# Avirup221/Multimodal-Hierarchical-CNN-for-Sun-Salutation-Pose-Classification

Hardware: AMD Instinct MI355X
Metric: images/sec fwd+bwd QuadtreeCNN 224x224 bs256 (higher is better)
Workload: dtype bf16; 1 GPU; QuadtreeCNN (ResNet-18 layer3, 2x2 split, 47-feat fusion) train step fwd+bwd+Adam, all parameters trainable; Adam(lr 1e-4, wd 1e-4) by the package's FusedAdam (csrc/pack.hip); global_batch=256, per_gpu_batch=256, image=3x224x224, num_classes=12, parallelism=dp1

## Files before the change

include/qtcnn.h:

```cpp
#ifndef QTCNN_H_
#define QTCNN_H_

#include <stddef.h>
#include <stdint.h>

#ifdef __cplusplus
extern "C" {
#endif

typedef enum qt_status {
  QT_OK = 0,
  QT_ERR_INVALID_ARG = -1,
  QT_ERR_LAUNCH = -2,
  QT_ERR_UNSUPPORTED = -3
} qt_status;

typedef enum qt_dtype { QT_F32 = 0, QT_BF16 = 1 } qt_dtype;

int qt_version(void);
const char* qt_last_error(void);

enum { QT_CONV_FWD = 0, QT_CONV_DGRAD = 1 };

typedef struct qt_conv_desc {
// ... 398 lines not shown
int qt_pack_dgrad_s2_merged(int dtype, const float* w_oihw, void* dst, int O, int I, void* stream);
int qt_pack_stem_weight(int dtype, const float* w_oihw, void* dst, int taps, void* stream);
int qt_unpack_conv_wgrad(const float* dw, float* grad_oihw, int O, int I, int kh, int kw, int accumulate, void* stream);
int qt_unpack_stem_wgrad(const float* dw, float* grad_oihw, int accumulate, void* stream);

int qt_stats_capacity_rows(int rows);
int qt_bn_finalize(float* partial, int rows, int C, long long count, const float* gamma, const float* beta,
                   float* running_mean, float* running_var, long long* num_batches_tracked, float momentum, float eps,
                   float* mean, float* invstd, float* scale, float* shift, void* stream);
int qt_bn_eval_affine(const float* gamma, const float* beta, const float* running_mean, const float* running_var,
                      float eps, int C, float* scale, float* shift, void* stream);
typedef struct qt_bn_eval_item {
  const float *gamma, *beta, *running_mean, *running_var;
  float *scale, *shift;
  int C;
  float *mean, *invstd;
} qt_bn_eval_item;
int qt_bn_eval_affine_batched(const qt_bn_eval_item* items, int n, float eps, void* stream);
int qt_bn_act(int dtype, const void* y, const float* scale, const float* shift, const void* residual,
              const float* res_scale, const float* res_shift, int relu, void* out, long long M, int C, void* stream);
int qt_bn_act_mask(int dtype, const void* y, const float* scale, const float* shift, const void* residual,
                   const float* res_scale, const float* res_shift, int relu, void* out, unsigned char* mask_bits,
                   long long M, int C, void* stream);
int qt_bn_bwd_partial_rows(long long M, int C);
int qt_bn_bwd_reduce(int dtype, const void* g, const void* mask, const void* y, const float* mean, const float* invstd,
                     float* partial, long long M, int C, void* stream);
int qt_bn_bwd_finalize(float* partial, int rows, int C, long long count, const float* gamma, const float* invstd,
                       float* dgamma, float* dbeta, int accumulate, float* coef , void* stream);
int qt_bn_bwd_apply(int dtype, const void* g, const void* mask, const void* y, const float* mean, const float* invstd,
                    const float* coef, void* dy, void* g_out, long long M, int C, void* stream);

int qt_stem_pool(int dtype, const void* y, const float* scale, const float* shift, void* pooled,
                 unsigned char* argmax, void* y_at_max, int batch, void* stream);
int qt_stem_conv_pool(int dtype, const void* xpad, const void* weight, int taps, const float* scale, const float* shift,
                      void* pooled, int batch, void* stream);
int qt_stem_conv_pool_nchw(int dtype, const float* image_nchw, const void* weight, int taps, const float* scale,
                           const float* shift, void* pooled, int batch, void* stream);
int qt_stem_pool_bwd(int dtype, const void* dpooled, const unsigned char* argmax, const void* y, const float* scale,
                     const float* shift, void* g, int batch, void* stream);
int qt_stem_bn_bwd_rows(int batch);
int qt_stem_bn_bwd_reduce(int dtype, const void* dpooled, const unsigned char* argmax, const void* y,
                          const float* scale, const float* shift, const float* mean, const float* invstd,
                          float* partial, int batch, void* stream);
int qt_stem_bn_bwd_sums_rows(int batch);
int qt_stem_bn_bwd_sums(int dtype, const void* dpooled, const void* y_at_max, const float* scale, const float* shift,
                        const float* mean, const float* invstd, float* partial, int batch, void* stream);
int qt_stem_bn_bwd_apply(int dtype, const void* dpooled, const unsigned char* argmax, const void* y, const float* scale,
                         const float* shift, const float* mean, const float* invstd, const float* coef, void* dy,
                         int batch, void* stream);
size_t qt_stem_bn_bwd_wgrad_workspace_bytes(int batch);
int qt_stem_bn_bwd_wgrad_ws(int dtype, const void* dpooled, const unsigned char* argmax, const void* y, const float* scale,
                            const float* shift, const float* mean, const float* invstd, const float* coef, const void* xpad,
                            float* dw, void* workspace, size_t workspace_bytes, int batch, void* stream);
int qt_stem_dgrad(int dtype, const void* dy, const float* w_oihw, float* dx, int batch, void* stream);
int qt_avgpool(int dtype, const void* x, void* dst, int batch, int hw, int C, int ld, int col0, void* stream);
int qt_avgpool_bwd(int dtype, const void* d, const void* x, void* g, int batch, int hw, int C, int ld, int col0,
                   void* stream);
int qt_quad_pool(int dtype, const void* q, void* dst, int batch, int ld, int col0, void* stream);
int qt_quad_pool_bwd(int dtype, const void* d, const void* q, void* dq, int batch, int ld, int col0, void* stream);
int qt_region_avgpool(int dtype, const void* x, void* dst, int dst_dtype, int batch, int split, int hw, int C, int ld,
                      int col0, void* stream);
int qt_region_avgpool_bwd(int dtype, const void* d, int d_dtype, const void* x, void* g, int batch, int split, int hw,
                          int C, int ld, int col0, void* stream);
int qt_attention_gate(int dtype, const float* v, const float* w1, const float* b1, const float* w2, const float* b2,
                      float* act, float* alpha, void* out, int batch, int ld, int col0, void* stream);
int qt_attention_gate_bwd(int dtype, const void* d, const float* v, const float* act, const float* alpha, const float* w1,
                          const float* w2, float* ds, float* dpre, float* dv, int batch, int ld, int col0, void* stream);
int qt_relu_mask_cols(int dtype, const void* d, const void* act, float* out, long long rows, int cols, int ld, int col0,
                      float mul, void* stream);
int qt_lstm_forward(const float* xproj, const float* whh_t, const float* bhh, float* gates, float* cell, float* hprev,
// ... 139 lines not shown
```

multimodal-hierarchical-cnn-for-sun-salutation-pose-classification_amd/csrc/conv_stem.hip:

```cpp
#include <stdlib.h>

#include "qt_internal.h"

namespace {

struct StemArgs {
  const bf16_t* x;
  const bf16_t* w;
  bf16_t* y;
  const float* scale;
  const float* shift;
  float* stats;
  int relu, taps, ntiles;
};

constexpr int ST_TH = 4;
constexpr int ST_ROWB = QT_STEM_PAD_W * 4 * 2;
constexpr int ST_IN_ROWS = 2 * ST_TH + 5;
constexpr int ST_BUF = 24 * 1024;
static_assert(ST_IN_ROWS * ST_ROWB <= ST_BUF, "a tile's input rows fit one buffer");
constexpr int ST_STG_ROW = 144;
constexpr int ST_STG = 16 * ST_STG_ROW;
constexpr int ST_LDS = 2 * ST_BUF + 4 * ST_STG;

template <bool AFF, bool STATS>
__global__ __launch_bounds__(256) void conv_stem_kernel(StemArgs p) {
  extern __shared__ __attribute__((aligned(16))) unsigned char smem[];
  const int tid = threadIdx.x, lane = tid & 63;
  const int wave = __builtin_amdgcn_readfirstlane(tid >> 6);
  const int li = lane & 15, lg = lane >> 4;
  const unsigned smem_base = lds_addr_of(smem);

  const int t_beg = (int)((long long)blockIdx.x * p.ntiles / gridDim.x);
  const int t_end = (int)((long long)(blockIdx.x + 1) * p.ntiles / gridDim.x);

  uint4 wf[7][4];
#pragma unroll
  for (int kh = 0; kh < 7; ++kh)
#pragma unroll
    for (int cb = 0; cb < 4; ++cb)
      wf[kh][cb] = *reinterpret_cast<const uint4*>(p.w + ((size_t)(cb * 16 + li) * p.taps + kh) * 32 + lg * 8);

  float sc[4][4], sh[4][4];
#pragma unroll
  for (int cb = 0; cb < 4; ++cb)
#pragma unroll
    for (int r = 0; r < 4; ++r) {
      const int ch = cb * 16 + lg * 4 + r;
      sc[cb][r] = p.scale ? p.scale[ch] : 1.f;
      sh[cb][r] = p.scale ? p.shift[ch] : 0.f;
    }
  float s1[4][4], s2[4][4];
#pragma unroll
  for (int cb = 0; cb < 4; ++cb)
#pragma unroll
    for (int r = 0; r < 4; ++r) s1[cb][r] = s2[cb][r] = 0.f;

  auto dma_tile = [&](int tile, int buf) {
    const int img = tile / 28, rg = tile - img * 28;
    const unsigned char* src = reinterpret_cast<const unsigned char*>(p.x) +
                               ((size_t)img * QT_STEM_PAD_H + (size_t)rg * 2 * ST_TH) * ST_ROWB;
#pragma unroll
    for (int i = 0; i < 6; ++i) {
      const int blk = wave * 6 + i;
      glds16(src + blk * 1024 + lane * 16, smem_base + buf * ST_BUF + blk * 1024);
    }
  };

  unsigned char* stg = smem + 2 * ST_BUF + wave * ST_STG;
  const unsigned keep8 = lg == 3 ? 0u : 0xffffffffu;
  if (t_beg < t_end) dma_tile(t_beg, 0);
  for (int t = t_beg; t < t_end; ++t) {
    const int buf = (t - t_beg) & 1;
    asm volatile("s_waitcnt vmcnt(0)\n\ts_barrier" ::: "memory");
    if (t + 1 < t_end) dma_tile(t + 1, buf ^ 1);
    const unsigned char* in = smem + buf * ST_BUF;
    const int img = t / 28, rg = t - img * 28;
#pragma unroll 1
    for (int j = 0; j < 7; ++j) {
      const int rb = wave + 4 * j;
      const int orow = rb / 7, ob = rb - orow * 7;
      const unsigned char* a0 = in + (2 * orow) * ST_ROWB + 16 * (ob * 16 + li + lg);
      uint4 xf[7];
#pragma unroll
      for (int kh = 0; kh < 7; ++kh) {
        xf[kh] = *reinterpret_cast<const uint4*>(a0 + kh * ST_ROWB);
        xf[kh].z &= keep8;
        xf[kh].w &= keep8;
      }
      f32x4 acc[4];
#pragma unroll
      for (int cb = 0; cb < 4; ++cb) acc[cb] = (f32x4){0.f, 0.f, 0.f, 0.f};
      __builtin_amdgcn_s_setprio(1);
#pragma unroll
      for (int kh = 0; kh < 7; ++kh)
#pragma unroll
        for (int cb = 0; cb < 4; ++cb)
          acc[cb] = __builtin_amdgcn_mfma_f32_16x16x32_bf16(__builtin_bit_cast(bf16x8, wf[kh][cb]),
                                                            __builtin_bit_cast(bf16x8, xf[kh]), acc[cb], 0, 0, 0);
      __builtin_amdgcn_s_setprio(0);
#pragma unroll
      for (int cb = 0; cb < 4; ++cb) {
        float v[4];
#pragma unroll
        for (int r = 0; r < 4; ++r) {
          const float a = acc[cb][r];
          if (STATS) {
            s1[cb][r] += a;
// ... 215 lines not shown
      auto max4 = [&](const uint4& a, const uint4& b) -> uint4 {
        return make_uint4(pkmax(a.x, b.x), pkmax(a.y, b.y), pkmax(a.z, b.z), pkmax(a.w, b.w));
      };
      const uint4 zero = make_uint4(0u, 0u, 0u, 0u);
      uint4 raw[5][3];
#pragma unroll
      for (int tr = 0; tr < 5; ++tr)
#pragma unroll
        for (int dc = 0; dc < 3; ++dc) {
          const int col = 2 * pw - 1 + dc;
          raw[tr][dc] = zero;
          if (!(k == 0 && tr == 0) && (unsigned)col < 112u)
            raw[tr][dc] = *reinterpret_cast<const uint4*>(ctile + (tr * 112 + col) * SP_PXB + cg * 16);
        }
      uint4 rowmax[5];
#pragma unroll
      for (int tr = 0; tr < 5; ++tr) rowmax[tr] = max4(max4(raw[tr][0], raw[tr][1]), raw[tr][2]);
#pragma unroll
      for (int pi = 0; pi < 2; ++pi) {
        const uint4 best = max4(max4(rowmax[2 * pi], rowmax[2 * pi + 1]), rowmax[2 * pi + 2]);
        *reinterpret_cast<uint4*>(p.pooled + (((size_t)img * 56 + 2 * k + pi) * 56 + pw) * 64 + cg * 8) = best;
      }
    }
  }
  asm volatile("s_waitcnt vmcnt(0)" ::: "memory");
}

int g_stem_enabled = -1;
bool stem_enabled() {
  if (g_stem_enabled < 0) g_stem_enabled = qt_env_int("QTCNN_STEM_CONV", 1);
  return g_stem_enabled != 0;
}

int stem_grid(int batch) {
  const int ntiles = batch * (112 / ST_TH);
  return ntiles < 512 ? ntiles : 512;
}

}

extern "C" void qt_set_stem_conv(int mode) { g_stem_enabled = mode < 0 ? 1 : (mode != 0); }

bool qt_stem_eligible(const qt_conv_desc* d, const qt_conv_io* io) {
  if (!stem_enabled() || d->dtype != QT_BF16 || d->mode != QT_CONV_FWD) return false;
  if (d->k_per_tap != 32 || d->kw != 1 || (d->kh != 7 && d->kh != 8) || d->stride != 2 || d->pad != 0) return false;
  if (d->n_out != 64 || d->out_h != 112 || d->out_w != 112 || d->in_h != QT_STEM_PAD_H || d->in_w != QT_STEM_PAD_W)
    return false;
  if (d->src_pix_stride != 4 || d->src_row_stride != QT_STEM_PAD_W * 4 ||
      d->src_img_stride != (long long)QT_STEM_PAD_H * QT_STEM_PAD_W * 4)
    return false;
  if (d->quad || d->dst_sub) return false;
  if (io && (io->residual || io->relu_mask || io->relu_mask_bits || io->bwd_bn[0].y || io->bwd_bn[1].y)) return false;
  return true;
}

int qt_stem_stats_rows(const qt_conv_desc* d) { return stem_grid(d->batch); }

int qt_stem_launch(const qt_conv_desc* d, const qt_conv_io* io, void* stream) {
  QT_CHECK_ARG((io->scale == nullptr) == (io->shift == nullptr), "qt_conv2d_igemm: scale and shift come together");
  StemArgs a;
  a.x = static_cast<const bf16_t*>(io->src);
  a.w = static_cast<const bf16_t*>(io->weight);
  a.y = static_cast<bf16_t*>(io->dst);
  a.scale = io->scale; a.shift = io->shift; a.stats = io->stats_partial;
  a.relu = d->relu; a.taps = d->kh; a.ntiles = d->batch * (112 / ST_TH);
  const bool aff = a.scale != nullptr || a.relu, stats = a.stats != nullptr;
  void (*kern)(StemArgs) = aff ? (stats ? conv_stem_kernel<true, true> : conv_stem_kernel<true, false>)
                               : (stats ? conv_stem_kernel<false, true> : conv_stem_kernel<false, false>);
  static std::atomic<unsigned long long> lds_limit_set[4];
  const int ki = (aff ? 2 : 0) + (stats ? 1 : 0);
  if (int rc = qt_raise_lds_limit(reinterpret_cast<const void*>(kern), ST_LDS, lds_limit_set[ki])) return rc;
  hipLaunchKernelGGL(kern, dim3(stem_grid(d->batch)), dim3(256), ST_LDS, static_cast<hipStream_t>(stream), a);
  QT_CHECK_LAUNCH();
  return QT_OK;
}

extern "C" int qt_stem_conv_pool(int dtype, const void* xpad, const void* weight, int taps, const float* scale,
                                 const float* shift, void* pooled, int batch, void* stream) {
  QT_CHECK_ARG(xpad && weight && scale && shift && pooled && batch > 0 && (taps == 7 || taps == 8),
               "qt_stem_conv_pool: bad argument");
  if (dtype != QT_BF16 || !stem_enabled()) {
    qt_set_error("qt_stem_conv_pool: bf16 only (use qt_conv2d_igemm + qt_stem_pool)");
    return QT_ERR_UNSUPPORTED;
  }
  StemPoolArgs a;
  a.x = static_cast<const bf16_t*>(xpad); a.w = static_cast<const bf16_t*>(weight); a.img = nullptr;
  a.pooled = static_cast<bf16_t*>(pooled); a.scale = scale; a.shift = shift; a.taps = taps; a.ntiles = batch * 28;
  static std::atomic<unsigned long long> lds_limit_set{0};
  if (int rc = qt_raise_lds_limit(reinterpret_cast<const void*>(conv_stem_pool_kernel<false>), SP_LDS, lds_limit_set)) return rc;
  const int grid = a.ntiles < 256 ? a.ntiles : 256;
  hipLaunchKernelGGL(conv_stem_pool_kernel<false>, dim3(grid), dim3(512), SP_LDS, static_cast<hipStream_t>(stream), a);
  QT_CHECK_LAUNCH();
  return QT_OK;
}

extern "C" int qt_stem_conv_pool_nchw(int dtype, const float* image_nchw, const void* weight, int taps, const float* scale,
                                      const float* shift, void* pooled, int batch, void* stream) {
  QT_CHECK_ARG(image_nchw && weight && scale && shift && pooled && batch > 0 && (taps == 7 || taps == 8),
               "qt_stem_conv_pool_nchw: bad argument");
  static const int raw_on = qt_env_int("QTCNN_STEM_NCHW", 1);
  if (dtype != QT_BF16 || !stem_enabled() || !raw_on || ((uintptr_t)image_nchw % 16) != 0) {
    qt_set_error("qt_stem_conv_pool_nchw: bf16 and a 16-byte aligned image only (use qt_pack_stem_input + qt_stem_conv_pool)");
    return QT_ERR_UNSUPPORTED;
  }
  StemPoolArgs a;
  a.x = nullptr; a.img = image_nchw; a.w = static_cast<const bf16_t*>(weight);
  a.pooled = static_cast<bf16_t*>(pooled); a.scale = scale; a.shift = shift; a.taps = taps; a.ntiles = batch * 28;
  static std::atomic<unsigned long long> lds_limit_set{0};
  if (int rc = qt_raise_lds_limit(reinterpret_cast<const void*>(conv_stem_pool_kernel<true>), SP_LDS_RAW, lds_limit_set)) return rc;
// ... 6 lines not shown
```

multimodal-hierarchical-cnn-for-sun-salutation-pose-classification_amd/csrc/elementwise.hip:

```cpp
#include "qt_common.h"

namespace {

__device__ __forceinline__ void load8f(const float* p, float (&v)[8]) { QtVec8<float>::load(p, v); }

constexpr int kFinC = 16;

__device__ __forceinline__ void sum_partial_rows(const float* __restrict__ partial, int rows, int C, int c, int rl,
                                                 double& s1, double& s2) {
  int r = rl;
  for (; r + 16 * 7 < rows; r += 16 * 8) {
    float a[8], b[8];
#pragma unroll
    for (int k = 0; k < 8; ++k) {
      a[k] = partial[((long long)(r + 16 * k) * 2 + 0) * C + c];
      b[k] = partial[((long long)(r + 16 * k) * 2 + 1) * C + c];
    }
#pragma unroll
    for (int k = 0; k < 8; ++k) {
      s1 += (double)a[k];
      s2 += (double)b[k];
    }
  }
  for (; r < rows; r += 16) {
// ... 325 lines not shown
      braw[e] = 0.f;
      bidx[e] = 0;
    }
#pragma unroll
    for (int kh = 0; kh < 3; ++kh) {
      const int h = ph * 2 - 1 + kh;
      if ((unsigned)h >= (unsigned)H) continue;
#pragma unroll
      for (int kw = 0; kw < 3; ++kw) {
        const int w = pw * 2 - 1 + kw;
        if ((unsigned)w >= (unsigned)W) continue;
        float v[8];
        QtVec8<T>::load(y + (((long long)n * H + h) * W + w) * C + c0, v);
#pragma unroll
        for (int e = 0; e < 8; ++e) {
          const float a = qt_relu(v[e] * sc[e] + sh[e]);
          if (qt_pool_wins(a, best[e])) {
            best[e] = a;
            braw[e] = v[e];
            bidx[e] = kh * 3 + kw;
          }
        }
      }
    }
    const long long off = (((long long)n * PH + ph) * PW + pw) * C + c0;
    QtVec8<T>::store(pooled + off, best);
    if (argmax) {
      uint2 pk;
      pk.x = bidx[0] | (bidx[1] << 8) | (bidx[2] << 16) | (bidx[3] << 24);
      pk.y = bidx[4] | (bidx[5] << 8) | (bidx[6] << 16) | (bidx[7] << 24);
      *reinterpret_cast<uint2*>(argmax + off) = pk;
    }
    if (y_at_max) QtVec8<T>::store(y_at_max + off, braw);
  }
}

template <typename T>
__global__ __launch_bounds__(256) void stem_bn_bwd_apply2x2_kernel(
    const T* __restrict__ dpooled, const unsigned char* __restrict__ argmax, const T* __restrict__ y,
    const float* __restrict__ scale, const float* __restrict__ shift, const float* __restrict__ mean,
    const float* __restrict__ invstd, const float* __restrict__ coef, T* __restrict__ out, int batch) {
  constexpr int H = 112, W = 112, C = 64, PH = 56, PW = 56;
  const long long total = (long long)batch * PH * PW * (C / 8);
  const int c0 = (int)((blockIdx.x * (long long)blockDim.x + threadIdx.x) % (C / 8)) * 8;
  float sc[8], sh[8], mu[8], is[8], ca[8], cb[8], cc[8];
  load8f(scale + c0, sc);
  load8f(shift + c0, sh);
  load8f(mean + c0, mu);
  load8f(invstd + c0, is);
  load8f(coef + c0, ca);
  load8f(coef + C + c0, cb);
  load8f(coef + 2 * C + c0, cc);
  for (long long i = blockIdx.x * (long long)blockDim.x + threadIdx.x; i < total;
       i += (long long)gridDim.x * blockDim.x) {
    const int b = (int)((i / (C / 8)) % PW);
    const int a = (int)((i / ((C / 8) * PW)) % PH);
    const int n = (int)(i / ((long long)(C / 8) * PW * PH));
    const bool a1 = a + 1 < PH, b1 = b + 1 < PW;
    const long long cell = (((long long)n * PH + a) * PW + b) * C + c0;
    uint2 k00 = *reinterpret_cast<const uint2*>(argmax + cell), k01 = make_uint2(0xffffffffu, 0xffffffffu), k10 = k01, k11 = k01;
    float d00[8], d01[8], d10[8], d11[8];
    QtVec8<T>::load(dpooled + cell, d00);
#pragma unroll
    for (int e = 0; e < 8; ++e) d01[e] = d10[e] = d11[e] = 0.f;
    if (b1) {
      k01 = *reinterpret_cast<const uint2*>(argmax + cell + C);
// ... 338 lines not shown
  const long long r0 = (long long)blockIdx.y * rows_per_block;
  long long r1 = r0 + rows_per_block;
  if (r1 > rows) r1 = rows;
  float s = 0.f;
  if (c < cols)
    for (long long r = r0 + rl; r < r1; r += 4) s += qt_to_f32<T>(x[r * ld + c]);
  red[rl][cl] = s;
  __syncthreads();
  if (rl == 0 && c < cols) {
    const float v = red[0][cl] + red[1][cl] + red[2][cl] + red[3][cl];
    if (part) part[(long long)blockIdx.y * cols + c] = v;
    else atomicAdd(out + c, v);
  }
}

__global__ __launch_bounds__(1024) void col_sum_finish_kernel(const float* __restrict__ part, int nparts, int cols,
                                                              float* __restrict__ out, int accumulate) {
  __shared__ float red[16][64];
  const int cl = threadIdx.x & 63, rl = threadIdx.x >> 6;
  const int c = blockIdx.x * 64 + cl;
  float s = 0.f;
  if (c < cols)
    for (int b = rl; b < nparts; b += 16) s += part[(long long)b * cols + c];
  red[rl][cl] = s;
  __syncthreads();
  if (rl == 0 && c < cols) {
    float v = 0.f;
#pragma unroll
    for (int l = 0; l < 16; ++l) v += red[l][cl];
    out[c] = accumulate ? out[c] + v : v;
  }
}

}

static int fold_partial(float*& partial, int& rows, int C, hipStream_t s) {
  if (rows <= 1024) return QT_OK;
  const int S = qt_cdiv(rows, kFold);
  hipLaunchKernelGGL(stats_stage1_kernel, dim3(qt_cdiv(C, 64), S), dim3(256), 0, s, partial, rows, C);
  QT_CHECK_LAUNCH();
  partial += (long long)rows * 2 * C;
  rows = S;
  return QT_OK;
}

extern "C" int qt_stats_capacity_rows(int rows) { return rows <= 1024 ? rows : rows + qt_cdiv(rows, kFold); }

extern "C" int qt_bn_finalize(float* partial, int rows, int C, long long count, const float* gamma,
                              const float* beta, float* running_mean, float* running_var,
                              long long* num_batches_tracked, float momentum, float eps, float* mean, float* invstd,
                              float* scale, float* shift, void* stream) {
  QT_CHECK_ARG(partial && rows > 0 && C > 0 && count > 0 && mean && invstd && scale && shift,
               "qt_bn_finalize: bad argument");
  QT_CHECK_ARG((running_mean == nullptr) == (running_var == nullptr), "qt_bn_finalize: running stats must come in pairs");
  if (int st = fold_partial(partial, rows, C, static_cast<hipStream_t>(stream))) return st;
  hipLaunchKernelGGL(bn_finalize_kernel, dim3(qt_cdiv(C, kFinC)), dim3(16 * kFinC), 0, static_cast<hipStream_t>(stream), partial,
                     rows, C, (double)count, gamma, beta, running_mean, running_var, num_batches_tracked, momentum, eps,
                     mean, invstd, scale, shift);
  QT_CHECK_LAUNCH();
  return QT_OK;
}

extern "C" int qt_bn_eval_affine(const float* gamma, const float* beta, const float* running_mean,
                                 const float* running_var, float eps, int C, float* scale, float* shift, void* stream) {
  QT_CHECK_ARG(gamma && beta && running_mean && running_var && scale && shift && C > 0, "qt_bn_eval_affine: bad argument");
  hipLaunchKernelGGL(bn_eval_affine_kernel, dim3(qt_cdiv(C, 256)), dim3(256), 0, static_cast<hipStream_t>(stream), gamma,
                     beta, running_mean, running_var, eps, C, scale, shift);
// ... 85 lines not shown
  return QT_OK;
}

extern "C" int qt_bn_bwd_apply(int dtype, const void* g, const void* mask, const void* y, const float* mean,
                               const float* invstd, const float* coef, void* dy, void* g_out, long long M, int C,
                               void* stream) {
  QT_DT_OK(dtype, "qt_bn_bwd_apply");
  QT_CHECK_ARG(g && y && mean && invstd && coef && dy && M > 0 && C > 0 && C % 8 == 0, "qt_bn_bwd_apply: bad argument");
  hipStream_t s = static_cast<hipStream_t>(stream);
  const int grid = qt_grid_for(M * (C / 8), 256, 16384);
  static const int light = qt_env_int("QTCNN_BN_APPLY_LIGHT", 1);
  const int cgs = C / 4;
  const int lgrid = qt_grid_for(M * cgs, 256, 16384);
  if (light && dtype == QT_BF16 && !mask && !g_out && ((long long)lgrid * 256) % cgs == 0 && M * cgs < (1ll << 29)) {
    hipLaunchKernelGGL(bn_bwd_apply_light_kernel, dim3(lgrid), dim3(256), 0, s, (const bf16_t*)g, (const bf16_t*)y, mean, invstd, coef,
                       (bf16_t*)dy, M * cgs, cgs, C);
    QT_CHECK_LAUNCH();
    return QT_OK;
  }
  qt_by_dtype(dtype, [&](auto* t) {
    using T = QT_T(t);
    hipLaunchKernelGGL(bn_bwd_apply_kernel<T>, dim3(grid), dim3(256), 0, s, qt_as<T>(g), qt_as<T>(mask), qt_as<T>(y), mean,
                       invstd, coef, qt_as<T>(dy), qt_as<T>(g_out), M, C);
  });
  QT_CHECK_LAUNCH();
  return QT_OK;
}

extern "C" int qt_stem_pool(int dtype, const void* y, const float* scale, const float* shift, void* pooled,
                            unsigned char* argmax, void* y_at_max, int batch, void* stream) {
  QT_DT_OK(dtype, "qt_stem_pool");
  QT_CHECK_ARG(y && scale && shift && pooled && batch > 0, "qt_stem_pool: bad argument");
  hipStream_t s = static_cast<hipStream_t>(stream);
  const int grid = qt_grid_for((long long)batch * 56 * 56 * 8, 256, 16384);
  qt_by_dtype(dtype, [&](auto* t) {
    using T = QT_T(t);
    hipLaunchKernelGGL(stem_pool_kernel<T>, dim3(grid), dim3(256), 0, s, qt_as<T>(y), scale, shift, qt_as<T>(pooled), argmax,
                       qt_as<T>(y_at_max), batch);
  });
  QT_CHECK_LAUNCH();
  return QT_OK;
}

template <typename T>
static void launch_stem_bwd(int mode, int grid, hipStream_t s, const void* dpooled, const unsigned char* argmax,
                            const void* y, const float* scale, const float* shift, const float* mean,
                            const float* invstd, const float* coef, float* partial, void* out, int batch) {
  if (mode == 0)
    hipLaunchKernelGGL((stem_pool_bwd_kernel<T, 0>), dim3(grid), dim3(256), 0, s, (const T*)dpooled, argmax, (const T*)y,
                       scale, shift, mean, invstd, coef, partial, (T*)out, batch);
  else if (mode == 1)
    hipLaunchKernelGGL((stem_pool_bwd_kernel<T, 1>), dim3(grid), dim3(256), 0, s, (const T*)dpooled, argmax, (const T*)y,
                       scale, shift, mean, invstd, coef, partial, (T*)out, batch);
  else
    hipLaunchKernelGGL((stem_pool_bwd_kernel<T, 2>), dim3(grid), dim3(256), 0, s, (const T*)dpooled, argmax, (const T*)y,
                       scale, shift, mean, invstd, coef, partial, (T*)out, batch);
}

extern "C" int qt_stem_pool_bwd(int dtype, const void* dpooled, const unsigned char* argmax, const void* y,
                                const float* scale, const float* shift, void* g, int batch, void* stream) {
  QT_DT_OK(dtype, "qt_stem_pool_bwd");
  QT_CHECK_ARG(dpooled && argmax && y && scale && shift && g && batch > 0, "qt_stem_pool_bwd: bad argument");
  hipStream_t s = static_cast<hipStream_t>(stream);
  const int grid = qt_grid_for((long long)batch * 112 * 112 * 8, 256, 16384);
  qt_by_dtype(dtype, [&](auto* t) {
    using T = QT_T(t);
// ... 268 lines not shown
```

multimodal-hierarchical-cnn-for-sun-salutation-pose-classification_amd/csrc/plan.hip:

```cpp
#include <stdlib.h>
#include <string.h>

#include <algorithm>
#include <string>
#include <vector>

#include "qt_common.h"

static bool merged_s2_enabled() {
  static const bool on = qt_env_int("QTCNN_S2_DGRAD_MERGED", 1) != 0;
  return on;
}

static bool ds_slot_enabled() {
  static const bool on = qt_env_int("QTCNN_DS_SLOT", 1) != 0;
  return on;
}

namespace {

constexpr int kImg = 224;

struct TensorInfo {
  std::string name;
// ... 818 lines not shown

  void quad_branch() {
    const ConvL& cq = p->convs[p->quad_conv];
    igemm(quad_desc(QT_CONV_FWD), at(p->blocks[5].out), at(cq.w_fwd), at(p->q), nullptr, tf(cq.bias), nullptr, nullptr,
          nullptr, 1);
    run(qt_quad_pool(dt, at(p->q), at(p->fused), B, p->fused_ld, 512, stream));
  }
  void mlp_branch() {
    const LinL& m0 = p->mlp0;
    const LinL& m1 = p->mlp1;
    dense_fwd(numerical, QT_F32, tf(m0.w), tf(m0.b), at(p->h1), QT_F32, B, m0.in, m0.out, 1, m0.in, m0.out, stream);
    if (dropout() && !p->lstm)
      run(qt_dropout(QT_F32, at(p->h1), B, m0.out, m0.out, seed, p->d.dropout_p, stream));
    dense_fwd(at(p->h1), QT_F32, tf(m1.w), tf(m1.b), at<unsigned char>(p->fused) + (size_t)p->mlp_col0 * p->esz, dt, B, m1.in,
              m1.out, 0, m1.in, p->fused_ld, stream);
  }
  void attn_branch() {
    const ConvL& cq = p->convs[p->quad_conv];
    const ConvL& cs = p->convs[p->sub_conv];
    const LinL& m0 = p->mlp0;
    const void* base = at(p->blocks[3].out);
    igemm(region_desc(cq, 2, QT_CONV_FWD), base, at(cq.w_fwd), at(cq.y), nullptr, tf(cq.bias), nullptr, nullptr, nullptr, 1);
    run(qt_region_avgpool(dt, at(cq.y), at(p->fused), dt, B, 2, 196, 128, p->fused_ld, 512, stream));
    igemm(region_desc(cs, 4, QT_CONV_FWD), base, at(cs.w_fwd), at(cs.y), nullptr, tf(cs.bias), nullptr, nullptr, nullptr, 1);
    run(qt_region_avgpool(dt, at(cs.y), at(p->vsub), QT_F32, B, 4, 49, 64, 16 * 64, 0, stream));
    run(qt_attention_gate(dt, at<float>(p->vsub), tf(p->att0.w), tf(p->att0.b), tf(p->att2.w), tf(p->att2.b),
                          at<float>(p->att_act), at<float>(p->att_alpha), at(p->fused), B, p->fused_ld, 512 + 4 * 128,
                          stream));
    unsigned char* z = at<unsigned char>(p->fused) + (size_t)p->mlp_col0 * p->esz;
    dense_fwd(numerical, QT_F32, tf(m0.w), tf(m0.b), z, dt, B, m0.in, m0.out, 1, m0.in, p->fused_ld, stream);
    if (dropout()) run(qt_dropout(dt, z, B, m0.out, p->fused_ld, seed, p->d.dropout_p, stream));
  }

  void stem() {
    const ConvL& c0 = p->convs[0];
    const BnL& bn0 = p->bns[c0.bn];
    const qt_conv_desc sd = stem_desc();
    int fused = QT_ERR_UNSUPPORTED;
    if (!unf) {
      const int slot = begin_timed(conv_flops(sd), 0, nullptr, (double)B * (3.0 * 224 * 224 * 4 + p->esz * 56.0 * 56 * 64));
      fused = qt_stem_conv_pool_nchw(dt, image, at(c0.w_fwd), stem_taps(), at<float>(bn0.scale), at<float>(bn0.shift),
                                     at(p->p0), B, stream);
      end_timed(slot);
      if (fused != QT_ERR_UNSUPPORTED) run(fused);
    }
    if (fused == QT_ERR_UNSUPPORTED) run(qt_pack_stem_input(dt, image, at(p->xpad), B, stream));
    if (fused == QT_ERR_UNSUPPORTED) conv_bn_stats(c0, sd, at(p->xpad), training);
    if (unf) {
      run(qt_stem_pool(dt, at(c0.y), at<float>(bn0.scale), at<float>(bn0.shift), at(p->p0), at<unsigned char>(p->argmax),
                       at(p->ymax), B, stream));
    } else if (fused == QT_ERR_UNSUPPORTED) {
      const int slot = begin_timed(conv_flops(sd), 0, nullptr,
                                   (double)B * p->esz * ((double)QT_STEM_PAD_H * QT_STEM_PAD_W * 4 + 56.0 * 56 * 64));
      fused = qt_stem_conv_pool(dt, at(p->xpad), at(c0.w_fwd), stem_taps(), at<float>(bn0.scale), at<float>(bn0.shift),
                                at(p->p0), B, stream);
      end_timed(slot);
      if (fused == QT_ERR_UNSUPPORTED) {
        igemm(sd, at(p->xpad), at(c0.w_fwd), at(c0.y), at<float>(bn0.scale), at<float>(bn0.shift), nullptr, nullptr, nullptr, 1);
        run(qt_stem_pool(dt, at(c0.y), at<float>(p->ones), at<float>(p->zeros), at(p->p0), nullptr, nullptr, B, stream));
      } else {
        run(fused);
      }
    }
  }

  void bn_relu(const ConvL& c, const qt_conv_desc& d, const void* src, const void* res, const BnL* res_bn, size_t out,
               size_t out_bits, bool conv_in_eval = true) {
    const BnL& bn = p->bns[c.bn];
    if (unf)
      run(qt_bn_act_mask(dt, at(c.y), at<float>(bn.scale), at<float>(bn.shift), res, res_bn ? at<float>(res_bn->scale) : nullptr,
                         res_bn ? at<float>(res_bn->shift) : nullptr, 1, at(out), at<unsigned char>(out_bits),
                         rows_of(c), c.cout, stream));
    else if (conv_in_eval)
      igemm(d, src, at(c.w_fwd), at(out), at<float>(bn.scale), at<float>(bn.shift), res, nullptr, nullptr, 1);
  }

  void blocks() {
    size_t x = p->p0;
    for (const Block& blk : p->blocks) {
      const ConvL& c1 = p->convs[blk.conv1];
      const ConvL& c2 = p->convs[blk.conv2];
      const qt_conv_desc d1 = conv_desc(c1, QT_CONV_FWD), d2 = conv_desc(c2, QT_CONV_FWD);
      const bool pair = blk.ds >= 0 && transition_pair(blk, at(x), training);
      if (blk.ds >= 0 && !pair) {
        const ConvL& cd = p->convs[blk.ds];
        const BnL& bd = p->bns[cd.bn];
        const qt_conv_desc dd = conv_desc(cd, QT_CONV_FWD);
        fork();
        on_side(p->stats_ds, [&] {
          conv_bn_stats(cd, dd, at(x), training);
          if (!unf)
            igemm(dd, at(x), at(cd.w_fwd), at(cd.y), at<float>(bd.scale), at<float>(bd.shift), nullptr, nullptr, nullptr, 0);
        });
      }
      if (!pair) conv_bn_stats(c1, d1, at(x), training);
      bn_relu(c1, d1, at(x), nullptr, nullptr, blk.a1, blk.a1_bits, !pair);
      conv_bn_stats(c2, d2, at(blk.a1), training);
      if (blk.ds >= 0) {
        const ConvL& cd = p->convs[blk.ds];
        if (!pair) join();
        bn_relu(c2, d2, at(blk.a1), at(cd.y), unf ? &p->bns[cd.bn] : nullptr, blk.out, blk.out_bits);
      } else {
        bn_relu(c2, d2, at(blk.a1), at(x), nullptr, blk.out, blk.out_bits);
      }
      x = blk.out;
      if (&blk == &p->blocks[p->attention ? 3 : 5] && !p->standard) {
        fork();
        on_side(p->stats_ds, [&] {
          if (p->attention) {
            attn_branch();
          } else {
            quad_branch();
            if (p->has_numerical && !mlp_early) mlp_branch();
          }
        });
      }
    }
    run(qt_avgpool(dt, at(p->blocks[7].out), at(p->fused), B, 49, 512, p->fused_ld, 0, stream));
  }

  void lstm_tail() {
    const int T = p->seq_len, S = B / T, H = p->lstm_h;
    for (int l = 0; l < 2 && ok(); ++l) {
      const qt_plan::LstmL& L = p->lstm_l[l];
      if (l == 0) run(qt_cast_f32(dt, at(p->fused), at<float>(p->lstm_x0), (long long)B * L.in, stream));
      igemm(dense_f32(B, L.in, 4 * H), l == 0 ? at(p->lstm_x0) : at(p->lstm_x1), tf(L.w_ih), at(L.xproj), nullptr, tf(L.b_ih),
            nullptr, nullptr, nullptr, 0);
      run(qt_transpose_f32(tf(L.w_hh), at<float>(L.whh_t), 4 * H, H, stream));
      run(qt_lstm_forward(at<float>(L.xproj), at<float>(L.whh_t), tf(L.b_hh), at<float>(L.gates), at<float>(L.cell),
                          at<float>(L.hprev), at<float>(L.hout), S, T, H, stream));
      if (l == 0) {
        hip(hipMemcpyAsync(at(p->lstm_x1), at(L.hout), (size_t)B * H * 4, hipMemcpyDeviceToDevice,
                           static_cast<hipStream_t>(stream)), "hipMemcpyAsync");
        if (dropout())
          run(qt_dropout(QT_F32, at(p->lstm_x1), B, H, H, seed ^ 0x3C3C3C3CC3C3C3C3ull, p->d.dropout_p, stream));
      }
    }
    const float* last = at<float>(p->lstm_l[1].hout) + (size_t)(T - 1) * H;
// ... 561 lines not shown
extern "C" int qt_plan_num_tensors(const qt_plan* p) { return p ? (int)p->tensors.size() : QT_ERR_INVALID_ARG; }
extern "C" const char* qt_plan_tensor_name(const qt_plan* p, int i) {
  return (p && i >= 0 && i < (int)p->tensors.size()) ? p->tensors[i].name.c_str() : nullptr;
}
extern "C" int qt_plan_tensor_kind(const qt_plan* p, int i) {
  return (p && i >= 0 && i < (int)p->tensors.size()) ? p->tensors[i].kind : QT_ERR_INVALID_ARG;
}
extern "C" int qt_plan_tensor_shape(const qt_plan* p, int i, int* dims) {
  if (!p || !dims || i < 0 || i >= (int)p->tensors.size()) return QT_ERR_INVALID_ARG;
  for (int k = 0; k < 4; ++k) dims[k] = p->tensors[i].shape[k];
  return p->tensors[i].ndim;
}
extern "C" size_t qt_plan_workspace_bytes(const qt_plan* p) { return p ? p->ws_bytes : 0; }

extern "C" int qt_plan_find_buffer(const qt_plan* p, const char* name, size_t* offset) {
  QT_CHECK_ARG(p && name && offset, "qt_plan_find_buffer: null argument");
  const std::string n(name);
  auto blockno = [&](const char* prefix) -> int {
    const size_t len = strlen(prefix);
    if (n.compare(0, len, prefix) != 0) return -1;
    return atoi(n.c_str() + len);
  };
  auto suffix = [&](const char* suf) {
    const size_t len = strlen(suf);
    return n.size() >= len && n.compare(n.size() - len, len, suf) == 0;
  };
  if (n == "fused") { *offset = p->fused; return QT_OK; }
  if (n == "dfused") { *offset = p->dfused; return QT_OK; }
  if (n == "hidden") { *offset = p->hidden; return QT_OK; }
  if (p->attention && n == "attention.vectors") { *offset = p->vsub; return QT_OK; }
  if (p->attention && n == "attention.weights") { *offset = p->att_alpha; return QT_OK; }
  if (n == "stem.pooled") { *offset = p->p0; return QT_OK; }
  if (n == "stem.gpooled") { *offset = p->g_p0; return QT_OK; }
  int b = blockno("block");
  if (b >= 0 && b < (int)p->blocks.size()) {
    const Block& blk = p->blocks[b];
    if (suffix(".out")) { *offset = blk.out; return QT_OK; }
    if (suffix(".gout")) { *offset = blk.gout; return QT_OK; }
    if (suffix(".a1")) { *offset = blk.a1; return QT_OK; }
  }
  int c = blockno("conv");
  if (c >= 0 && c < (int)p->convs.size()) {
    if (suffix(".y")) { *offset = p->convs[c].y; return QT_OK; }
    if (suffix(".gy")) { *offset = p->convs[c].gy; return QT_OK; }
  }
  qt_set_error("qt_plan_find_buffer: unknown buffer '%s'", name);
  return QT_ERR_INVALID_ARG;
}

extern "C" int qt_plan_profile_begin(qt_plan* p) {
  QT_CHECK_ARG(p, "qt_plan_profile_begin: null plan");
  for (auto& t : p->timed) { (void)hipEventDestroy(t.a); (void)hipEventDestroy(t.b); }
  p->timed.clear();
  p->profiling = true;
  return QT_OK;
}
extern "C" int qt_plan_profile_end(qt_plan* p, double* flops, double* ms, int* launches) {
  QT_CHECK_ARG(p && flops && ms && launches, "qt_plan_profile_end: null argument");
  p->profiling = false;
  for (int k = 0; k < 3; ++k) { flops[k] = 0; ms[k] = 0; launches[k] = 0; p->last_profile_bytes[k] = 0; }
  int st = QT_OK;
  for (auto& t : p->timed) {
    float dt = 0.f;
    if (hipEventSynchronize(t.b) != hipSuccess || hipEventElapsedTime(&dt, t.a, t.b) != hipSuccess) {
      qt_set_error("qt_plan_profile_end: event query failed");
      st = QT_ERR_LAUNCH;
// ... 165 lines not shown
```

Baseline: 47030 images/s.

## Add row-walking stem maxpool kernel and optional raw-NCHW stem conv path

Adds a stem max-pool kernel in which each block walks a strip of output rows and carries the shared input row forward, so overlapping 3x3 windows are not reloaded from global memory. It is enabled by default through an env switch. Separately adds an opt-in stem conv kernel that reads the fp32 NCHW image directly into LDS, converts it to bf16 in place, and emits BN stats. This skips the packed-input step; the xpad pack is deferred to a side stream after layer1 for backward use. The raw path is disabled by default. It trades LDS occupancy and a single-buffered schedule for removing the pack pass from the critical path.

```diff
diff --git a/include/qtcnn.h b/include/qtcnn.h
--- a/include/qtcnn.h
+++ b/include/qtcnn.h
@@ -454,10 +454,14 @@
 
 int qt_stem_pool(int dtype, const void* y, const float* scale, const float* shift, void* pooled,
                  unsigned char* argmax, void* y_at_max, int batch, void* stream);
+void qt_set_stem_pool_walk(int mode);
 int qt_stem_conv_pool(int dtype, const void* xpad, const void* weight, int taps, const float* scale, const float* shift,
                       void* pooled, int batch, void* stream);
 int qt_stem_conv_pool_nchw(int dtype, const float* image_nchw, const void* weight, int taps, const float* scale,
                            const float* shift, void* pooled, int batch, void* stream);
+int qt_stem_conv_stats_nchw(int dtype, const float* image_nchw, const void* weight, int taps, void* y, float* stats,
+                            int batch, void* stream);
+void qt_set_stem_conv_raw(int mode);
 int qt_stem_pool_bwd(int dtype, const void* dpooled, const unsigned char* argmax, const void* y, const float* scale,
                      const float* shift, void* g, int batch, void* stream);
 int qt_stem_bn_bwd_rows(int batch);
diff --git a/multimodal-hierarchical-cnn-for-sun-salutation-pose-classification_amd/csrc/conv_stem.hip b/multimodal-hierarchical-cnn-for-sun-salutation-pose-classification_amd/csrc/conv_stem.hip
--- a/multimodal-hierarchical-cnn-for-sun-salutation-pose-classification_amd/csrc/conv_stem.hip
+++ b/multimodal-hierarchical-cnn-for-sun-salutation-pose-classification_amd/csrc/conv_stem.hip
@@ -12,6 +12,7 @@
   const float* shift;
   float* stats;
   int relu, taps, ntiles;
+  const float* img;
 };
 
 constexpr int ST_TH = 4;
@@ -22,8 +23,12 @@
 constexpr int ST_STG_ROW = 144;
 constexpr int ST_STG = 16 * ST_STG_ROW;
 constexpr int ST_LDS = 2 * ST_BUF + 4 * ST_STG;
-
-template <bool AFF, bool STATS>
+constexpr int ST_RAW_ROWS = 3 * ST_IN_ROWS;
+constexpr int ST_RAW_STG = ST_RAW_ROWS * 1024;
+constexpr int ST_LDS_RAW = ST_BUF + ST_RAW_STG + 4 * ST_STG;
+static_assert(2 * ST_LDS_RAW <= 160 * 1024, "two raw-input workgroups per CU");
+
+template <bool AFF, bool STATS, bool RAW = false>
 __global__ __launch_bounds__(256) void conv_stem_kernel(StemArgs p) {
   extern __shared__ __attribute__((aligned(16))) unsigned char smem[];
   const int tid = threadIdx.x, lane = tid & 63;
@@ -67,13 +72,72 @@
     }
   };
 
-  unsigned char* stg = smem + 2 * ST_BUF + wave * ST_STG;
+  auto dma_raw = [&](int tile) {
+    const int img = tile / 28, rg = tile - img * 28;
+#pragma unroll
+    for (int i = 0; i < 10; ++i) {
+      const int r = wave + 4 * i;
+      if (r < ST_RAW_ROWS) {
+        const int c = r / ST_IN_ROWS, j = r - c * ST_IN_ROWS;
+        const int h = 8 * rg - 3 + j;
+        if ((unsigned)h < 224u && lane < 56)
+          glds16(p.img + (((size_t)img * 3 + c) * 224 + h) * 224 + lane * 4, smem_base + ST_BUF + r * 1024);
+      }
+    }
+  };
+  auto convert_raw = [&](int tile) {
+    const int rg = tile % 28;
+    f32x4 v[3][3];
+#pragma unroll
+    for (int r = 0; r < 3; ++r) {
+      const int it = tid + r * 256;
+      const int j = it / 56, g = it - j * 56;
+      const int h = 8 * rg - 3 + j;
+#pragma unroll
+      for (int c = 0; c < 3; ++c) v[r][c] = (f32x4){0.f, 0.f, 0.f, 0.f};
+      if (it < ST_IN_ROWS * 56 && (unsigned)h < 224u) {
+        const unsigned char* s0 = smem + ST_BUF + j * 1024 + g * 16;
+#pragma unroll
+        for (int c = 0; c < 3; ++c) v[r][c] = *reinterpret_cast<const f32x4*>(s0 + c * ST_IN_ROWS * 1024);
+      }
+    }
+#pragma unroll
+    for (int r = 0; r < 3; ++r) {
+      const int it = tid + r * 256;
+      const int j = it / 56, g = it - j * 56;
+      if (it < ST_IN_ROWS * 56) {
+        unsigned char* d = smem + j * ST_ROWB + (4 * g + 3) * 8;
+#pragma unroll
+        for (int q = 0; q < 4; ++q) {
+          const bf16x4 o = {(bf16_t)v[r][0][q], (bf16_t)v[r][1][q], (bf16_t)v[r][2][q], (bf16_t)0.f};
+          *reinterpret_cast<bf16x4*>(d + q * 8) = o;
+        }
+      }
+    }
+    if (tid < ST_IN_ROWS * 8) {
+      const int j = tid >> 3, b = tid & 7;
+      const bf16x4 z = {(bf16_t)0.f, (bf16_t)0.f, (bf16_t)0.f, (bf16_t)0.f};
+      *reinterpret_cast<bf16x4*>(smem + j * ST_ROWB + (b < 3 ? b : 224 + b) * 8) = z;
+    }
+  };
+
+  unsigned char* stg = smem + (RAW ? ST_BUF + ST_RAW_STG : 2 * ST_BUF) + wave * ST_STG;
   const unsigned keep8 = lg == 3 ? 0u : 0xffffffffu;
-  if (t_beg < t_end) dma_tile(t_beg, 0);
+  if (t_beg < t_end) {
+    if constexpr (RAW) dma_raw(t_beg);
+    else dma_tile(t_beg, 0);
+  }
   for (int t = t_beg; t < t_end; ++t) {
-    const int buf = (t - t_beg) & 1;
-    asm volatile("s_waitcnt vmcnt(0)\n\ts_barrier" ::: "memory");
-    if (t + 1 < t_end) dma_tile(t + 1, buf ^ 1);
+    const int buf = RAW ? 0 : (t - t_beg) & 1;
+    if constexpr (RAW) {
+      asm volatile("s_waitcnt vmcnt(0) lgkmcnt(0)\n\ts_barrier" ::: "memory");
+      convert_raw(t);
+      asm volatile("s_waitcnt lgkmcnt(0)\n\ts_barrier" ::: "memory");
+      if (t + 1 < t_end) dma_raw(t + 1);
+    } else {
+      asm volatile("s_waitcnt vmcnt(0)\n\ts_barrier" ::: "memory");
+      if (t + 1 < t_end) dma_tile(t + 1, buf ^ 1);
+    }
     const unsigned char* in = smem + buf * ST_BUF;
     const int img = t / 28, rg = t - img * 28;
 #pragma unroll 1
@@ -355,6 +419,9 @@
   return g_stem_enabled != 0;
 }
 
+constexpr int kStemRawDefault = 0;
+int g_stem_raw = -1;
+
 int stem_grid(int batch) {
   const int ntiles = batch * (112 / ST_TH);
   return ntiles < 512 ? ntiles : 512;
@@ -363,6 +430,7 @@
 }
 
 extern "C" void qt_set_stem_conv(int mode) { g_stem_enabled = mode < 0 ? 1 : (mode != 0); }
+extern "C" void qt_set_stem_conv_raw(int mode) { g_stem_raw = mode < 0 ? kStemRawDefault : (mode != 0); }
 
 bool qt_stem_eligible(const qt_conv_desc* d, const qt_conv_io* io) {
   if (!stem_enabled() || d->dtype != QT_BF16 || d->mode != QT_CONV_FWD) return false;
@@ -386,7 +454,7 @@
   a.w = static_cast<const bf16_t*>(io->weight);
   a.y = static_cast<bf16_t*>(io->dst);
   a.scale = io->scale; a.shift = io->shift; a.stats = io->stats_partial;
-  a.relu = d->relu; a.taps = d->kh; a.ntiles = d->batch * (112 / ST_TH);
+  a.relu = d->relu; a.taps = d->kh; a.ntiles = d->batch * (112 / ST_TH); a.img = nullptr;
   const bool aff = a.scale != nullptr || a.relu, stats = a.stats != nullptr;
   void (*kern)(StemArgs) = aff ? (stats ? conv_stem_kernel<true, true> : conv_stem_kernel<true, false>)
                                : (stats ? conv_stem_kernel<false, true> : conv_stem_kernel<false, false>);
@@ -398,6 +466,26 @@
   return QT_OK;
 }
 
+extern "C" int qt_stem_conv_stats_nchw(int dtype, const float* image_nchw, const void* weight, int taps, void* y, float* stats,
+                                       int batch, void* stream) {
+  QT_CHECK_ARG(image_nchw && weight && y && stats && batch > 0 && (taps == 7 || taps == 8),
+               "qt_stem_conv_stats_nchw: bad argument");
+  if (g_stem_raw < 0) g_stem_raw = qt_env_int("QTCNN_STEM_CONV_RAW", kStemRawDefault) != 0;
+  if (dtype != QT_BF16 || !stem_enabled() || !g_stem_raw || ((uintptr_t)image_nchw % 16) != 0) {
+    qt_set_error("qt_stem_conv_stats_nchw: bf16 and a 16-byte aligned image only (use qt_pack_stem_input + qt_conv2d_igemm)");
+    return QT_ERR_UNSUPPORTED;
+  }
+  StemArgs a;
+  a.x = nullptr; a.img = image_nchw; a.w = static_cast<const bf16_t*>(weight); a.y = static_cast<bf16_t*>(y);
+  a.scale = nullptr; a.shift = nullptr; a.stats = stats; a.relu = 0; a.taps = taps; a.ntiles = batch * (112 / ST_TH);
+  void (*kern)(StemArgs) = conv_stem_kernel<false, true, true>;
+  static std::atomic<unsigned long long> lds_limit_set{0};
+  if (int rc = qt_raise_lds_limit(reinterpret_cast<const void*>(kern), ST_LDS_RAW, lds_limit_set)) return rc;
+  hipLaunchKernelGGL(kern, dim3(stem_grid(batch)), dim3(256), ST_LDS_RAW, static_cast<hipStream_t>(stream), a);
+  QT_CHECK_LAUNCH();
+  return QT_OK;
+}
+
 extern "C" int qt_stem_conv_pool(int dtype, const void* xpad, const void* weight, int taps, const float* scale,
                                  const float* shift, void* pooled, int batch, void* stream) {
   QT_CHECK_ARG(xpad && weight && scale && shift && pooled && batch > 0 && (taps == 7 || taps == 8),
diff --git a/multimodal-hierarchical-cnn-for-sun-salutation-pose-classification_amd/csrc/elementwise.hip b/multimodal-hierarchical-cnn-for-sun-salutation-pose-classification_amd/csrc/elementwise.hip
--- a/multimodal-hierarchical-cnn-for-sun-salutation-pose-classification_amd/csrc/elementwise.hip
+++ b/multimodal-hierarchical-cnn-for-sun-salutation-pose-classification_amd/csrc/elementwise.hip
@@ -381,6 +381,97 @@
       *reinterpret_cast<uint2*>(argmax + off) = pk;
     }
     if (y_at_max) QtVec8<T>::store(y_at_max + off, braw);
+  }
+}
+
+template <typename T> struct QtRaw8;
+template <> struct QtRaw8<bf16_t> {
+  uint4 u;
+  __device__ __forceinline__ void load(const bf16_t* p) { u = *reinterpret_cast<const uint4*>(p); }
+  __device__ __forceinline__ void get(float (&v)[8]) const {
+    v[0] = __uint_as_float(u.x << 16); v[1] = __uint_as_float(u.x & 0xffff0000u);
+    v[2] = __uint_as_float(u.y << 16); v[3] = __uint_as_float(u.y & 0xffff0000u);
+    v[4] = __uint_as_float(u.z << 16); v[5] = __uint_as_float(u.z & 0xffff0000u);
+    v[6] = __uint_as_float(u.w << 16); v[7] = __uint_as_float(u.w & 0xffff0000u);
+  }
+};
+template <> struct QtRaw8<float> {
+  float4 a, b;
+  __device__ __forceinline__ void load(const float* p) {
+    a = *reinterpret_cast<const float4*>(p);
+    b = *reinterpret_cast<const float4*>(p + 4);
+  }
+  __device__ __forceinline__ void get(float (&v)[8]) const {
+    v[0] = a.x; v[1] = a.y; v[2] = a.z; v[3] = a.w;
+    v[4] = b.x; v[5] = b.y; v[6] = b.z; v[7] = b.w;
+  }
+};
+
+constexpr int kStemPoolWalkThreads = 56 * 8;
+
+template <typename T>
+__global__ __launch_bounds__(kStemPoolWalkThreads) void stem_pool_walk_kernel(
+    const T* __restrict__ y, const float* __restrict__ scale, const float* __restrict__ shift, T* __restrict__ pooled,
+    unsigned char* __restrict__ argmax, T* __restrict__ y_at_max, int strip, int strips) {
+  constexpr int H = 112, W = 112, C = 64, PH = 56, PW = 56;
+  const int n = blockIdx.x / strips, s = blockIdx.x - n * strips;
+  const int c0 = (threadIdx.x & 7) * 8, pw = threadIdx.x >> 3;
+  const int ph0 = s * strip, ph1 = ph0 + strip < PH ? ph0 + strip : PH;
+  const bool left = pw > 0;
+  float sc[8], sh[8];
+  load8f(scale + c0, sc);
+  load8f(shift + c0, sh);
+  const T* col = y + ((long long)n * H * W + (2 * pw - 1)) * C + c0;
+  auto load_row = [&](int h, QtRaw8<T> (&r)[3]) {
+    const T* p = col + (long long)h * W * C;
+    if (left) r[0].load(p);
+    r[1].load(p + C);
+    r[2].load(p + 2 * C);
+  };
+  QtRaw8<T> rows[3][3] = {};
+  if (ph0 > 0) load_row(2 * ph0 - 1, rows[0]);
+#pragma unroll 1
+  for (int ph = ph0; ph < ph1; ++ph) {
+    load_row(2 * ph, rows[1]);
+    load_row(2 * ph + 1, rows[2]);
+    float best[8], braw[8];
+    int bidx[8];
+#pragma unroll
+    for (int e = 0; e < 8; ++e) {
+      best[e] = -INFINITY;
+      braw[e] = 0.f;
+      bidx[e] = 0;
+    }
+#pragma unroll
+    for (int kh = 0; kh < 3; ++kh) {
+      if (kh == 0 && ph == 0) continue;
+#pragma unroll
+      for (int kw = 0; kw < 3; ++kw) {
+        if (kw == 0 && !left) continue;
+        float v[8];
+        rows[kh][kw].get(v);
+#pragma unroll
+        for (int e = 0; e < 8; ++e) {
+          const float a = qt_relu(v[e] * sc[e] + sh[e]);
+          if (qt_pool_wins(a, best[e])) {
+            best[e] = a;
+            braw[e] = v[e];
+            bidx[e] = kh * 3 + kw;
+          }
+        }
+      }
+    }
+    const long long off = (((long long)n * PH + ph) * PW + pw) * C + c0;
+    QtVec8<T>::store(pooled + off, best);
+    if (argmax) {
+      uint2 pk;
+      pk.x = bidx[0] | (bidx[1] << 8) | (bidx[2] << 16) | (bidx[3] << 24);
+      pk.y = bidx[4] | (bidx[5] << 8) | (bidx[6] << 16) | (bidx[7] << 24);
+      *reinterpret_cast<uint2*>(argmax + off) = pk;
+    }
+    if (y_at_max) QtVec8<T>::store(y_at_max + off, braw);
+#pragma unroll
+    for (int kw = 0; kw < 3; ++kw) rows[0][kw] = rows[2][kw];
   }
 }
 
@@ -785,7 +876,12 @@
   }
 }
 
-}
+int g_stem_pool_walk = -1;
+constexpr int kStemPoolStrip = 8;
+
+}
+
+extern "C" void qt_set_stem_pool_walk(int mode) { g_stem_pool_walk = mode < 0 ? 1 : (mode != 0); }
 
 static int fold_partial(float*& partial, int& rows, int C, hipStream_t s) {
   if (rows <= 1024) return QT_OK;
@@ -937,6 +1033,22 @@
   QT_DT_OK(dtype, "qt_stem_pool");
   QT_CHECK_ARG(y && scale && shift && pooled && batch > 0, "qt_stem_pool: bad argument");
   hipStream_t s = static_cast<hipStream_t>(stream);
+  if (g_stem_pool_walk < 0) g_stem_pool_walk = qt_env_int("QTCNN_STEM_POOL_WALK", 1) != 0;
+  if (g_stem_pool_walk) {
+    static const int strip = [] {
+      const int v = qt_env_int("QTCNN_STEM_POOL_STRIP", kStemPoolStrip);
+      return v < 1 ? 1 : (v > 56 ? 56 : v);
+    }();
+    const int strips = (56 + strip - 1) / strip;
+    QT_CHECK_ARG((long long)batch * strips < (1ll << 31), "qt_stem_pool: batch %d too large", batch);
+    qt_by_dtype(dtype, [&](auto* t) {
+      using T = QT_T(t);
+      hipLaunchKernelGGL(stem_pool_walk_kernel<T>, dim3(batch * strips), dim3(kStemPoolWalkThreads), 0, s, qt_as<T>(y), scale,
+                         shift, qt_as<T>(pooled), argmax, qt_as<T>(y_at_max), strip, strips);
+    });
+    QT_CHECK_LAUNCH();
+    return QT_OK;
+  }
   const int grid = qt_grid_for((long long)batch * 56 * 56 * 8, 256, 16384);
   qt_by_dtype(dtype, [&](auto* t) {
     using T = QT_T(t);
diff --git a/multimodal-hierarchical-cnn-for-sun-salutation-pose-classification_amd/csrc/plan.hip b/multimodal-hierarchical-cnn-for-sun-salutation-pose-classification_amd/csrc/plan.hip
--- a/multimodal-hierarchical-cnn-for-sun-salutation-pose-classification_amd/csrc/plan.hip
+++ b/multimodal-hierarchical-cnn-for-sun-salutation-pose-classification_amd/csrc/plan.hip
@@ -874,6 +874,14 @@
     if (dropout()) run(qt_dropout(dt, z, B, m0.out, p->fused_ld, seed, p->d.dropout_p, stream));
   }
 
+  bool pack_pending = false;
+  void pack_xpad_aside() {
+    if (!pack_pending) return;
+    pack_pending = false;
+    fork();
+    on_side(p->stats_ds, [&] { run(qt_pack_stem_input(dt, image, at(p->xpad), B, stream)); });
+  }
+
   void stem() {
     const ConvL& c0 = p->convs[0];
     const BnL& bn0 = p->bns[c0.bn];
@@ -886,8 +894,23 @@
       end_timed(slot);
       if (fused != QT_ERR_UNSUPPORTED) run(fused);
     }
-    if (fused == QT_ERR_UNSUPPORTED) run(qt_pack_stem_input(dt, image, at(p->xpad), B, stream));
-    if (fused == QT_ERR_UNSUPPORTED) conv_bn_stats(c0, sd, at(p->xpad), training);
+    bool raw_conv = false;
+    if (tr && unf && wstream && wstream != stream && ok()) {
+      float* part = at<float>(stats_off == (size_t)-1 ? p->stats : stats_off);
+      const int slot = begin_timed(conv_flops(sd), 0, nullptr,
+                                   (double)B * (3.0 * 224 * 224 * 4 + p->esz * 112.0 * 112 * 64) + 64.0 * stem_taps() * 32 * p->esz);
+      const int raw = qt_stem_conv_stats_nchw(dt, image, at(c0.w_fwd), stem_taps(), at(c0.y), part, B, stream);
+      end_timed(slot);
+      if (raw != QT_ERR_UNSUPPORTED) {
+        run(raw);
+        if (ok()) bn_finalize(bn0, part, qt_conv2d_stats_rows(&sd), rows_of(c0));
+        raw_conv = pack_pending = true;
+        static const bool right_away = qt_env_int("QTCNN_STEM_PACK_AFTER_LAYER1", 1) == 0;
+        if (right_away) pack_xpad_aside();
+      }
+    }
+    if (fused == QT_ERR_UNSUPPORTED && !raw_conv) run(qt_pack_stem_input(dt, image, at(p->xpad), B, stream));
+    if (fused == QT_ERR_UNSUPPORTED && !raw_conv) conv_bn_stats(c0, sd, at(p->xpad), training);
     if (unf) {
       run(qt_stem_pool(dt, at(c0.y), at<float>(bn0.scale), at<float>(bn0.shift), at(p->p0), at<unsigned char>(p->argmax),
                        at(p->ymax), B, stream));
@@ -946,6 +969,7 @@
         bn_relu(c2, d2, at(blk.a1), at(x), nullptr, blk.out, blk.out_bits);
       }
       x = blk.out;
+      if (&blk == &p->blocks[1]) pack_xpad_aside();
       if (&blk == &p->blocks[p->attention ? 3 : 5] && !p->standard) {
         fork();
         on_side(p->stats_ds, [&] {
@@ -1573,6 +1597,7 @@
   if (p->attention && n == "attention.weights") { *offset = p->att_alpha; return QT_OK; }
   if (n == "stem.pooled") { *offset = p->p0; return QT_OK; }
   if (n == "stem.gpooled") { *offset = p->g_p0; return QT_OK; }
+  if (n == "stem.xpad") { *offset = p->xpad; return QT_OK; }
   int b = blockno("block");
   if (b >= 0 && b < (int)p->blocks.size()) {
     const Block& blk = p->blocks[b];
```

After: 47020 images/s. No clear change (-0.0%).
